# Corv/CUDA-GMM-MPI

Measured on NVIDIA H100. Metric: EM iterations/sec at N=10M D=24 K=64; E-step HBM GB/s vs roofline, higher is better.
Workload: dtype f32

## Files before the change

cuda-gmm-mpi_b200/csrc/gmm_api.cu:

```cuda
#include <cuda_runtime.h>
#include <dlfcn.h>
#include <fcntl.h>
#include <unistd.h>
#include <nccl.h>

#include <algorithm>
#include <atomic>
#include <chrono>
#include <condition_variable>
#include <functional>
#include <mutex>
#include <cmath>
#include <cstdint>
#include <cstdio>
#include <cstdlib>
#include <cstring>
#include <limits>
#include <string>
#include <thread>
#include <vector>

#include "../../include/gmm.h"
#include "host_math.h"
#include "kernels_simt.cuh"
// ... 2671 lines not shown
    if (!c || !out) return fail(GMM_ERR_ARG, "gmm_get_profile: bad argument");
    cudaStreamSynchronize(c->stream);
    collect_all(c);
    out[0] = c->t_estep.total_ms; out[1] = c->t_mstep.total_ms; out[2] = c->host_const_ms;
    out[3] = c->t_reduce.total_ms; out[4] = c->memcpy_ms + c->t_final.total_ms; out[5] = (double)c->mstep_tensor;
    out[6] = (double)c->iterations; out[7] = (double)c->mstep_simt;
    if (reset) {
        c->t_estep.total_ms = c->t_mstep.total_ms = c->t_reduce.total_ms = c->t_fused.total_ms = 0;
        c->host_const_ms = c->memcpy_ms = 0; c->iterations = 0; c->t_final.total_ms = 0;
        c->mstep_tensor = c->mstep_simt = 0;
        c->fit_reduce_ms = c->fit_seed_ms = c->fit_save_ms = 0;
    }
    return GMM_OK;
}

int gmm_host_pool_selftest(int threads, int jobs, int n) {
    if (threads < 1 || jobs < 1 || n < 0) return fail(GMM_ERR_ARG, "gmm_host_pool_selftest: bad argument");
    HostPool pool(threads);
    std::vector<std::atomic<int>> hits((size_t)(n > 0 ? n : 1));
    for (auto& h : hits) h.store(0);
    for (int j = 0; j < jobs; j++) {
        const int m = (j % 3 == 0) ? n : (j % 3 == 1 ? (n + 1) / 2 : 1);
        const std::function<void(int)> fn = [&](int i) { hits[(size_t)i].fetch_add(1, std::memory_order_relaxed); };
        pool.run(m, fn);
        for (int i = 0; i < n; i++) {
            const int want = i < m ? 1 : 0;
            if (hits[(size_t)i].exchange(0) != want) return fail(GMM_ERR_STATE, "gmm_host_pool_selftest: an item ran the wrong number of times");
        }
        if (j % 64 == 63) pool.resize(1 + (j / 64) % threads);
        if (j % 200 == 199) std::this_thread::sleep_for(std::chrono::milliseconds(6));
// ... 71 lines not shown
```

cuda-gmm-mpi_b200/csrc/kernels_tc.cu:

```cuda
#include <cuda.h>
#include <cudaTypedefs.h>
#include <cuda_fp16.h>
#if defined(__F16C__) && defined(__AVX__)
#include <immintrin.h>
#endif
#include <cuda_runtime.h>

#include <cmath>
#include <cstdio>
#include <cstdlib>
#include <cstring>
#include <string>
#include <type_traits>
#include <vector>

#include "host_math.h"
#include "kernels_tc.cuh"
#include "mstep_rows.h"
#include "tc_ptx.cuh"

namespace gmm {

using namespace ptx;

// ... 14 lines not shown
constexpr float kGammaScale = 1024.0f;
constexpr float kGammaMagic = 1.5f * 134217728.0f;

template <int D, int NCL_> struct MCfg {
    static_assert(D % 4 == 0, "tensor M-step: D must be a multiple of 4");
    static_assert(NCL_ == 32 || NCL_ == 64, "tensor M-step: 32 or 64 clusters per CTA");
    static constexpr int NCL = NCL_;
    static constexpr int HPC = 64 / NCL;
    static constexpr int F = 1 + D + D * (D + 1) / 2;
    static constexpr int S = D / 4;
    static constexpr int MT = (4 * ((1 + 2 * S + S * (D / 2) + 7) / 8) * 8 + 127) / 128;
    static constexpr int G_PART = NCL * kTE * 2;
    static constexpr int G_STAGE = 3 * G_PART;
    static constexpr int RAWZ = (D * kTE * 4 + 1023) / 1024 * 1024;
    static constexpr int RAWX = RAWZ + 1024;
    static constexpr int RAWG = NCL * kTE * 4;
    static constexpr int OFF_G = 0;
    static constexpr int OFF_RAWX = OFF_G + kNST * G_STAGE;
    static constexpr int OFF_RAWG = OFF_RAWX + kNRAW * RAWX;
    static constexpr int NCT = MT * 128;
    static constexpr int OFF_RACC = OFF_RAWG + kNRAW * RAWG;
    static constexpr int OFF_BAR = OFF_RACC + 32 * NCT * 4;
    static constexpr int SMEM_BYTES = OFF_BAR + 512;
    static constexpr int THREADS = 128 + NCT;
    static constexpr int REG_LAUNCH = (65536 / THREADS) / 8 * 8 > 255 ? 255 : (65536 / THREADS) / 8 * 8;
    static constexpr int REG_P = MT == 1 ? REG_LAUNCH : 56;
    static constexpr int REG_C = MT == 3 ? 152 : (MT == 2 ? 224 : REG_LAUNCH);
    static_assert(128 * REG_P + NCT * REG_C <= THREADS * REG_LAUNCH, "register pools");
    static_assert(OFF_RAWX % 1024 == 0 && RAWX % 1024 == 0 && RAWZ % 1024 == 0, "SWIZZLE_128B TMA destinations need 1024-byte alignment");
    static_assert(OFF_RAWG % 1024 == 0 && RAWG % 1024 == 0, "SWIZZLE_128B TMA destinations need 1024-byte alignment");
    static_assert(MT <= 3, "feature tiles");
};

// ... 47 lines not shown
        lo[ks][2 * u + 1] = pack_half2(l2, l3);
#endif
    }
}

__device__ __forceinline__ void load_row(uint32_t addr, float2 (&z)[4]) {
#pragma unroll
    for (int p = 0; p < 4; p++) z[p] = lds_f2(addr ^ (uint32_t)(p << 5));
}

template <int NCL>
__device__ __forceinline__ void issue_half(float (&ex)[NCL / 2], float (&rm)[NCL / 2], const uint32_t (&hi)[2][4], const uint32_t (&lo)[2][4],
                                           uint32_t gam, bool new1, bool new2) {
#pragma unroll
    for (int ks = 0; ks < kTE / 16; ks++) {
        const uint64_t hdesc = make_smem_desc(gam + ks * 256,  128,  512);
        const uint64_t ldesc = make_smem_desc(gam + NCL * kTE * 2 + ks * 256, 128, 512);
        const uint64_t sdesc = make_smem_desc(gam + 2 * NCL * kTE * 2 + ks * 256, 128, 512);
#if GMM_MSTEP_CUT == 1
        asm volatile("" ::"r"(hi[ks][0]), "r"(hi[ks][1]), "r"(hi[ks][2]), "r"(hi[ks][3]), "r"(lo[ks][0]), "r"(lo[ks][1]), "r"(lo[ks][2]),
                     "r"(lo[ks][3]), "l"(hdesc), "l"(ldesc), "l"(sdesc));
        (void)ex; (void)rm; (void)new1; (void)new2;
#else
        if constexpr (NCL == 32) {
            wgmma_m64n32k16_rs(ex, hi[ks][0], hi[ks][1], hi[ks][2], hi[ks][3], hdesc, ks > 0 || !new1);
            wgmma_m64n32k16_rs(rm, hi[ks][0], hi[ks][1], hi[ks][2], hi[ks][3], ldesc, ks > 0 || !new2);
            wgmma_m64n32k16_rs(rm, lo[ks][0], lo[ks][1], lo[ks][2], lo[ks][3], sdesc, true);
        } else {
            wgmma_m64n64k16_rs(ex, hi[ks][0], hi[ks][1], hi[ks][2], hi[ks][3], hdesc, ks > 0 || !new1);
            wgmma_m64n64k16_rs(rm, hi[ks][0], hi[ks][1], hi[ks][2], hi[ks][3], ldesc, ks > 0 || !new2);
            wgmma_m64n64k16_rs(rm, lo[ks][0], lo[ks][1], lo[ks][2], lo[ks][3], sdesc, true);
        }
#endif
// ... 5 lines not shown
__device__ __forceinline__ bool chain2_ends(int i, int mt, int nsub) { return ((i + mt) % kChunkSub2) == kChunkSub2 - 1 || i == nsub - 1; }
__device__ __forceinline__ bool chain2_starts(int i, int mt) { return i == 0 || ((i + mt) % kChunkSub2) == 0; }

template <int D, int NCL, bool WT = false>
__global__ void __launch_bounds__(MCfg<D, NCL>::THREADS, 1)
mstep_tc_kernel(const __grid_constant__ CUtensorMap tm_x, const __grid_constant__ CUtensorMap tm_g, int n, int K,
                float* __restrict__ scratch, int events_per_cta, const __grid_constant__ MMagic magic, const int* __restrict__ opmap,
                const float* __restrict__ wts, float w_max, float w_inv) {
    using C = MCfg<D, NCL>;
    constexpr int HPC = C::HPC;
    extern __shared__ __align__(1024) uint8_t smem[];
    uint64_t* bars = reinterpret_cast<uint64_t*>(smem + C::OFF_BAR);
    uint64_t* raw_full = bars;
    uint64_t* raw_empty = bars + kNRAW;
    uint64_t* op_full = bars + 2 * kNRAW;
    uint64_t* op_empty = op_full + kNST;

    const int warp = threadIdx.x >> 5, lane = threadIdx.x & 31;
    const int range = blockIdx.x / (2 / HPC), part = blockIdx.x % (2 / HPC);
    const int e_begin = range * events_per_cta;
    const int e_end = min(n, e_begin + events_per_cta);
    const int nsub = (e_end - e_begin + kTE - 1) / kTE;
    const int k0 = blockIdx.y * NCL;

    for (int i = threadIdx.x; i < kNRAW * 256; i += C::THREADS)
        reinterpret_cast<float*>(smem + C::OFF_RAWX + (i >> 8) * C::RAWX + C::RAWZ)[i & 255] = 1.0f;
    if (threadIdx.x == 0) {
        for (int s = 0; s < kNRAW; s++) { mbar_init(&raw_full[s], 1); mbar_init(&raw_empty[s], 3 + 4 * C::MT); }
        for (int s = 0; s < kNST; s++) { mbar_init(&op_full[s], 3); mbar_init(&op_empty[s], 4 * C::MT); }
        fence_mbar_init();
    }
    __syncthreads();

    if (warp < 4) {
        set_regs<C::REG_P, C::REG_LAUNCH>();
        if (warp == 0) {
            const int nbox = min(NCL, K - k0 + kNCL - 1) / kNCL;
            if (elect_one()) {
                for (int i = 0; i < nsub; i++) {
                    const int st = i % kNRAW, ph = (i / kNRAW) & 1;
                    mbar_wait_parked(&raw_empty[st], ph ^ 1, 500);
                    mbar_arrive_expect_tx(&raw_full[st], kTE * D * 4 + nbox * kNCL * kTE * 4);
                    const int e0 = e_begin + i * kTE;
                    tma_load_2d(smem + C::OFF_RAWX + st * C::RAWX, &tm_x, e0, 0, &raw_full[st]);
                    for (int b = 0; b < nbox; b++)
                        tma_load_2d(smem + C::OFF_RAWG + st * C::RAWG + b * kNCL * kTE * 4, &tm_g, e0, k0 + b * kNCL, &raw_full[st]);
                }
            }
        } else {
            const int bt = threadIdx.x - 32;
            constexpr int NITEM = 4 * NCL, NIT = (NITEM + 95) / 96;
            for (int i = 0; i < nsub; i++) {
                const int rs = i % kNRAW, rph = (i / kNRAW) & 1;
                const int os = i % kNST, oph = (i / kNST) & 1;
                [[maybe_unused]] float wv[8];
                if constexpr (WT) {
                    const float4* wp = reinterpret_cast<const float4*>(wts + e_begin + i * kTE + 8 * ((bt & 31) >> 3));
                    const float4 wa = __ldg(wp), wb = __ldg(wp + 1);
                    wv[0] = wa.x; wv[1] = wa.y; wv[2] = wa.z; wv[3] = wa.w; wv[4] = wb.x; wv[5] = wb.y; wv[6] = wb.z; wv[7] = wb.w;
#pragma unroll
                    for (int v = 0; v < 8; v++) wv[v] = wv[v] == w_max ? 1.0f : __fmul_rn(wv[v], w_inv);
                }
                mbar_wait_parked(&raw_full[rs], rph, 200);
                mbar_wait_parked(&op_empty[os], oph ^ 1, 200);
                uint8_t* g_hi = smem + C::OFF_G + os * C::G_STAGE;
                float dep = 0.0f;
#pragma unroll
                for (int u = 0; u < NIT; u++) {
                    const int it = bt + 96 * u;
                    if (it >= NITEM) break;
                    const int kg = it >> 5, l = it & 31;
                    const int k = kg * 8 + (l & 7), ce = l >> 3;
                    const uint8_t* grow = smem + C::OFF_RAWG + rs * C::RAWG + k * (kTE * 4);
                    const float4 a = *reinterpret_cast<const float4*>(grow + (((2 * ce) ^ (k & 7)) << 4));
                    const float4 b = *reinterpret_cast<const float4*>(grow + (((2 * ce + 1) ^ (k & 7)) << 4));
                    float g[8] = {a.x, a.y, a.z, a.w, b.x, b.y, b.z, b.w};
                    dep += a.x + b.x;
                    if constexpr (WT) {
#pragma unroll
                        for (int v = 0; v < 8; v++) g[v] = __fmul_rn(g[v], wv[v]);
                    }
                    float hi[8], lo[8];
#pragma unroll
                    for (int v = 0; v < 8; v++) {
                        hi[v] = __fsub_rn(__fmaf_rn(g[v], kGammaScale, kGammaMagic), kGammaMagic);
// ... 51 lines not shown
            for (int j = 0; j < NCL / 2; j++) { ex[h][j] = 0.0f; rm[h][j] = 0.0f; }
        auto add_to_racc = [&](float (&acc)[HPC][NCL / 2]) {
#pragma unroll
            for (int c = 0; c < 2; c++) {
#pragma unroll
                for (int j = 0; j < 16; j++) {
                    const int q = 16 * c + j;
                    racc[q * C::NCT] += acc[q / (NCL / 2)][q % (NCL / 2)];
                }
                asm volatile("" ::: "memory");
            }
        };
        uint32_t fh[2][2][4], fl[2][2][4];
        float2 za[4];
        int held = -1;
        auto group = [&](int i, auto hc, uint32_t (&gh)[2][4], uint32_t (&gl)[2][4]) {
            constexpr int h = decltype(hc)::value;
            const int rs = i % kNRAW, rph = (i / kNRAW) & 1;
            const int os = i % kNST, oph = (i / kNST) & 1;
            const uint32_t zst = zs0 + rs * C::RAWX;
            const uint32_t gam = smem_u32(smem + C::OFF_G + os * C::G_STAGE);
            const bool new1 = chain_starts(i, mt), new2 = chain2_starts(i, mt);
            if constexpr (h == 0) {
                mbar_wait_parked(&raw_full[rs], rph, 100);
                load_row(zst + fa, za);
            }
            float2 zb0[4], zb1[4];
            load_row(zst + fb[2 * h], zb0);
            load_row(zst + fb[2 * h + 1], zb1);
            build_half(za, zb0, zb1, mg[2 * h], mg[2 * h + 1], gh, gl);
            if constexpr (h == 0) mbar_wait_parked(&op_full[os], oph, 100);
            wgmma_fence();
            issue_half<NCL>(ex[h], rm[h], gh, gl, gam, new1, new2);
            wgmma_commit();
            if constexpr (h == HPC - 1) {
                __syncwarp();
                if (lane == 0) mbar_arrive(&raw_empty[rs]);
            }
            wgmma_wait<1>();
            if constexpr (h == 0) {
                __syncwarp();
                if (lane == 0 && held >= 0) mbar_arrive(&op_empty[held]);
            }
            if constexpr (h == HPC - 1) {
                held = os;
                if (chain_ends(i, mt, nsub)) {
                    wgmma_wait<0>();
                    __syncwarp();
                    if (lane == 0) mbar_arrive(&op_empty[os]);
                    held = -1;
#if GMM_MSTEP_CUT != 3
                    add_to_racc(ex);
                    if (chain2_ends(i, mt, nsub)) add_to_racc(rm);
#endif
                }
            }
        };
        using H0 = std::integral_constant<int, 0>;
        using H1 = std::integral_constant<int, 1>;
        if constexpr (HPC == 2) {
            for (int i = 0; i < nsub; i++) {
                group(i, H0{}, fh[0], fl[0]);
                group(i, H1{}, fh[1], fl[1]);
            }
// ... 14 lines not shown
        add_to_racc(ex);
#endif
        const int nranges = gridDim.x * HPC / 2;
#pragma unroll
        for (int h = 0; h < HPC; h++)
#pragma unroll
            for (int j = 0; j < NCL / 2; j += 2) {
                const int q = h * (NCL / 2) + j;
                const int row = ((hx & 1) + h) * 64 + wq * 16 + gid + 8 * ((j >> 1) & 1);
                const int col = (j >> 2) * 8 + 2 * qd;
                const int ty = blockIdx.y * (NCL / kNCL) + col / kNCL;
                float* dst = scratch + ((((size_t)ty * nranges + range) * C::MT + mt) * 128 + row) * kNCL + col % kNCL;
                *reinterpret_cast<float2*>(dst) = make_float2(racc[q * C::NCT], racc[(q + 1) * C::NCT]);
            }
    }
}

__global__ void standardise_soa_kernel(const float* __restrict__ xs, float* __restrict__ zs, size_t pitch, int n, int D,
                                       const float* __restrict__ shift_f, const float* __restrict__ inv_scale_f) {
    const int d = blockIdx.y;
    const float s = shift_f[d], isc = inv_scale_f[d];
    const float* x = xs + (size_t)d * pitch;
    float* z = zs + (size_t)d * pitch;
    for (long long e = (long long)blockIdx.x * blockDim.x + threadIdx.x; e < n; e += (long long)gridDim.x * blockDim.x)
        z[e] = __fmul_rn(__fsub_rn(x[e], s), isc);
}

__global__ void __launch_bounds__(256)
mstep_tc_finalize_kernel(const float* __restrict__ scratch, int ncta_x, int MT, int K, int F, const int3* __restrict__ rowmap,
                         const double* __restrict__ scale, double* __restrict__ stats, double wscale) {
// ... 464 lines not shown
    bool emap_ok = false;
    uint8_t* d_bimg = nullptr;
    uint8_t* h_bimg = nullptr;
    size_t bimg_bytes = 0;
    uint8_t* d_opnd = nullptr;
    uint8_t* h_opnd = nullptr;
    cudaEvent_t ev_h2d = nullptr;
    bool h2d_pending = false;
    float* d_ck = nullptr;
    float* h_ck = nullptr;
    float* d_den = nullptr;
    int e_ck_len = 0;
    int e_NG = 0;
    int host_threads = 8;
    bool attr_estep = false, attr_mstep = false, attr_score = false;
    double h_shift[GMM_MAX_DIMENSIONS] = {0}, h_scale[GMM_MAX_DIMENSIONS] = {0};
};

static PFN_cuTensorMapEncodeTiled_v12000 encode_fn() {
    static PFN_cuTensorMapEncodeTiled_v12000 fn = nullptr;
    static bool tried = false;
    if (!tried) {
        tried = true;
        void* p = nullptr;
        cudaDriverEntryPointQueryResult q;
        if (cudaGetDriverEntryPoint("cuTensorMapEncodeTiled", &p, cudaEnableDefault, &q) == cudaSuccess && q == cudaDriverEntryPointSuccess)
            fn = reinterpret_cast<PFN_cuTensorMapEncodeTiled_v12000>(p);
    }
    return fn;
}
// ... 644 lines not shown
    return GMM_OK;
}

int tc_launch_score(TcState* t, int K, const TcScoreIo& io, cudaStream_t stream) {
    if (!t || !t->emap_ok) return fail(GMM_ERR_STATE, "tensor scoring not initialised for this shape");
    if (io.n <= 0) return GMM_OK;
    switch (t->D) {
        case 8: return launch_score_d<8>(t, K, io, stream);
        case 16: return launch_score_d<16>(t, K, io, stream);
        case 24: return launch_score_d<24>(t, K, io, stream);
        default: return fail(GMM_ERR_ARG, "tensor scoring: unsupported D");
    }
}

template <int D>
static int launch_mstep_d(TcState* t, int K, const CUtensorMap& tm_x, const CUtensorMap& tm_g, int n, double* d_stats, const float* w,
                          double wscale, cudaStream_t stream) {
    using C32 = MCfg<D, 32>;
    using C64 = MCfg<D, 64>;
    static_assert(C32::SMEM_BYTES <= 232448 && C64::SMEM_BYTES <= 232448, "shared memory budget");
    if (!t->attr_mstep) {
        TC_CUDA_TRY(cudaFuncSetAttribute(mstep_tc_kernel<D, 32>, cudaFuncAttributeMaxDynamicSharedMemorySize, C32::SMEM_BYTES));
        TC_CUDA_TRY(cudaFuncSetAttribute(mstep_tc_kernel<D, 64>, cudaFuncAttributeMaxDynamicSharedMemorySize, C64::SMEM_BYTES));
        TC_CUDA_TRY(cudaFuncSetAttribute(mstep_tc_kernel<D, 32, true>, cudaFuncAttributeMaxDynamicSharedMemorySize, C32::SMEM_BYTES));
        TC_CUDA_TRY(cudaFuncSetAttribute(mstep_tc_kernel<D, 64, true>, cudaFuncAttributeMaxDynamicSharedMemorySize, C64::SMEM_BYTES));
        t->attr_mstep = true;
    }
    const float w_max = (float)wscale, w_inv = (float)(1.0 / wscale);
    int gx = t->num_sms;
    int per = (n + gx - 1) / gx;
    per = (per + kTE - 1) / kTE * kTE;
    gx = (n + per - 1) / per;
    const bool pair = K > 32;
    const int ncl = pair ? 64 : 32;
    const int gy = (K + ncl - 1) / ncl;
    if ((size_t)gx * gy * (ncl / kNCL) * C32::MT * 128 * kNCL > t->scratch_floats) return fail(GMM_ERR_STATE, "tensor M-step scratch too small");
    const dim3 grid(pair ? 2 * gx : gx, gy);
    if (pair) {
        if (w) mstep_tc_kernel<D, 64, true><<<grid, C64::THREADS, C64::SMEM_BYTES, stream>>>(tm_x, tm_g, n, K, t->d_scratch, per, t->magic, t->d_opmap, w, w_max, w_inv);
        else mstep_tc_kernel<D, 64><<<grid, C64::THREADS, C64::SMEM_BYTES, stream>>>(tm_x, tm_g, n, K, t->d_scratch, per, t->magic, t->d_opmap, nullptr, 1.0f, 1.0f);
    } else {
        if (w) mstep_tc_kernel<D, 32, true><<<grid, C32::THREADS, C32::SMEM_BYTES, stream>>>(tm_x, tm_g, n, K, t->d_scratch, per, t->magic, t->d_opmap, w, w_max, w_inv);
        else mstep_tc_kernel<D, 32><<<grid, C32::THREADS, C32::SMEM_BYTES, stream>>>(tm_x, tm_g, n, K, t->d_scratch, per, t->magic, t->d_opmap, nullptr, 1.0f, 1.0f);
    }
    TC_CUDA_TRY(cudaGetLastError());
    mstep_tc_finalize_kernel<<<C32::MT * 128, 256, 0, stream>>>(t->d_scratch, gx, C32::MT, K, C32::F, t->d_rowmap, t->d_scale, d_stats,
                                                                w ? wscale : 1.0);
    TC_CUDA_TRY(cudaGetLastError());
    return GMM_OK;
}

static int launch_mstep_any(TcState* t, int K, const CUtensorMap& tm_x, const CUtensorMap& tm_g, int n, double* d_stats, const float* w,
                            double wscale, cudaStream_t stream) {
    if (!t || !t->maps_ok) return fail(GMM_ERR_STATE, "tensor-core M-step not initialised for this shape");
    if (!t->have_shift) return fail(GMM_ERR_STATE, "tensor-core M-step needs gmm_seed (shift/scale) first");
// ... 16 lines not shown

int tc_launch_mstep_on(TcState* t, int K, const float* d_z, const float* d_memb, size_t pitch, int n, double* d_stats, cudaStream_t stream) {
    if (n <= 0) return GMM_OK;
    if (!t || !t->maps_ok) return fail(GMM_ERR_STATE, "tensor-core M-step not initialised for this shape");
    if (t->cmap_z != d_z || t->cmap_g != d_memb || t->cmap_pitch != pitch || t->cmap_n != n) {
        t->cmap_n = -1;
        if (int rc = make_map_2d(&t->tm_cx, d_z, (uint64_t)n, (uint64_t)t->D, (uint64_t)pitch * 4, kTE, (uint32_t)t->D, true)) return rc;
        if (int rc = make_map_2d(&t->tm_cg, d_memb, (uint64_t)n, (uint64_t)t->Kmax, (uint64_t)pitch * 4, kTE, kNCL, true)) return rc;
        t->cmap_z = d_z; t->cmap_g = d_memb; t->cmap_pitch = pitch; t->cmap_n = n;
    }
    return launch_mstep_any(t, K, t->tm_cx, t->tm_cg, n, d_stats, nullptr, 1.0, stream);
}

const float* tc_shift_f(const TcState* t) { return t && t->have_shift ? t->d_shift_f : nullptr; }
const float* tc_inv_scale_f(const TcState* t) { return t && t->have_shift ? t->d_inv_scale_f : nullptr; }
float tc_mstep_zbound(const TcState* t) {
    float zb = 0.f;
    if (t)
        for (int d = 0; d < t->D; d++) zb = std::fmax(zb, t->zmax[d]);
    return zb;
}

}
```

cuda-gmm-mpi_b200/csrc/kernels_tc.cuh:

```cuda
#pragma once
#include <cuda_runtime.h>
#include "../../include/gmm.h"

namespace gmm {

struct TcState;

bool tc_mstep_supported(int D, int K);
bool tc_estep_supported(int D, int K);

int  tc_create(TcState** out, const float* d_x_aos, const float* d_x_soa, int n, int D, int Kmax, float* d_memb, size_t memb_pitch,
               int num_sms, cudaStream_t stream);
void tc_destroy(TcState*);
void tc_set_host_threads(TcState*, int n);
int  tc_set_shift_scale(TcState*, double* shift, const double* scale, const double* xmin, const double* xmax, cudaStream_t stream);
bool tc_mstep_ready(const TcState*);
bool tc_estep_range_ok(const TcState*);
int  tc_upload_params(TcState*, const clusters_t* host, int K, cudaStream_t stream);
int  tc_params_begin(TcState*, int K, cudaStream_t stream);
int  tc_params_padded(const TcState*, int K);
int  tc_params_cluster(TcState*, const clusters_t* host, int k, int K);
int  tc_params_cluster_w(TcState*, const clusters_t* host, int k, int K, const double* W);
int  tc_params_commit(TcState*, int K, int bad, cudaStream_t stream);
int  tc_launch_estep(TcState*, int K, double* d_ll, cudaStream_t stream, const float* d_w = nullptr);
// ... 11 lines not shown
};
int  tc_launch_score(TcState*, int K, const TcScoreIo& io, cudaStream_t stream);
bool tc_finalize_supported(const TcState*, int K);
size_t tc_param_set_floats(int Kmax, int D);
size_t tc_param_set_off(int Kmax, int D, int which);
int  tc_launch_finalize(TcState*, int K, const double* d_stats, const float* d_avgvar, float* d_set, double* d_ll, int* d_bad, int iter,
                        int fault_iter, cudaStream_t stream);
int  tc_launch_mstep(TcState*, int K, double* d_stats, cudaStream_t stream, const float* d_w = nullptr, double wscale = 1.0);

int  tc_launch_estep_on(TcState*, int K, const float* d_x_aos, int n, float* d_memb, size_t pitch, float* d_den, double* d_ll,
                        cudaStream_t stream);
int  tc_launch_mstep_on(TcState*, int K, const float* d_z, const float* d_memb, size_t pitch, int n, double* d_stats, cudaStream_t stream);
const float* tc_shift_f(const TcState*);
const float* tc_inv_scale_f(const TcState*);
float tc_mstep_zbound(const TcState*);

}
```

cuda-gmm-mpi_b200/csrc/tc_ptx.cuh:

```cuda
#pragma once
#include <cuda_runtime.h>
#include <cstdint>

namespace gmm { namespace ptx {

__device__ __forceinline__ uint32_t smem_u32(const void* p) {
    return static_cast<uint32_t>(__cvta_generic_to_shared(p));
}

__device__ __forceinline__ void mbar_init(uint64_t* bar, uint32_t count) {
    asm volatile("mbarrier.init.shared::cta.b64 [%0], %1;" ::"r"(smem_u32(bar)), "r"(count) : "memory");
}
__device__ __forceinline__ void fence_mbar_init() {
    asm volatile("fence.mbarrier_init.release.cluster;" ::: "memory");
}
__device__ __forceinline__ void mbar_arrive(uint64_t* bar) {
    asm volatile("mbarrier.arrive.shared::cta.b64 _, [%0];" ::"r"(smem_u32(bar)) : "memory");
}
__device__ __forceinline__ void mbar_arrive_after(uint64_t* bar, float dep) {
    asm volatile(
        "{\n\t.reg .pred p;\n\t.reg .b32 cnt;\n\t"
        "setp.ne.b32 p, %1, 0xff800001;\n\t"
        "selp.b32 cnt, 1, 2, p;\n\t"
        "mbarrier.arrive.shared::cta.b64 _, [%0], cnt;\n\t}"
// ... 12 lines not shown
    return ok != 0;
}
__device__ __forceinline__ void mbar_wait(uint64_t* bar, uint32_t parity) {
    while (!mbar_try_wait(bar, parity)) {}
}
__device__ __forceinline__ void mbar_wait_parked(uint64_t* bar, uint32_t parity, uint32_t ns) {
    uint32_t ok = 0;
    while (!ok) {
        asm volatile(
            "{\n\t.reg .pred p;\n\t"
            "mbarrier.try_wait.parity.shared::cta.b64 p, [%1], %2, %3;\n\t"
            "selp.u32 %0, 1, 0, p;\n\t}"
            : "=r"(ok) : "r"(smem_u32(bar)), "r"(parity), "r"(ns) : "memory");
    }
}
__device__ __forceinline__ void fence_proxy_async_smem() {
    asm volatile("fence.proxy.async.shared::cta;" ::: "memory");
}

__device__ __forceinline__ void tma_load_1d(void* smem_dst, const void* gmem_src, uint32_t bytes, uint64_t* bar) {
    asm volatile(
        "cp.async.bulk.shared::cluster.global.mbarrier::complete_tx::bytes [%0], [%1], %2, [%3];"
        ::"r"(smem_u32(smem_dst)), "l"(gmem_src), "r"(bytes), "r"(smem_u32(bar)) : "memory");
}

__device__ __forceinline__ uint64_t make_smem_desc(uint32_t saddr, uint32_t lbo_bytes, uint32_t sbo_bytes) {
    uint64_t d = 0;
    d |= (uint64_t)((saddr >> 4) & 0x3FFF);
    d |= (uint64_t)((lbo_bytes >> 4) & 0x3FFF) << 16;
    d |= (uint64_t)((sbo_bytes >> 4) & 0x3FFF) << 32;
// ... 71 lines not shown
```

cuda-gmm-mpi_b200/engine.py:

```python
import ctypes as C
import os
import subprocess

import numpy as np

from .clusters import Clusters, clusters_t

_HERE = os.path.dirname(os.path.abspath(__file__))
_FP = C.POINTER(C.c_float)
_DP = C.POINTER(C.c_double)
_IP = C.POINTER(C.c_int)
_CP = C.POINTER(clusters_t)

PATH_AUTO, PATH_SIMT, PATH_TENSOR = 0, 1, 2
VB_DIRICHLET_PROCESS, VB_DIRICHLET_DISTRIBUTION = 0, 1


class gmm_vb_prior(C.Structure):
    _fields_ = [("weight_prior_type", C.c_int), ("weight_concentration", C.c_double), ("mean_precision", C.c_double),
                ("dof", C.c_double), ("mean", _DP), ("covariance", _DP), ("reg_covar", C.c_double)]


class gmm_vb_posterior(C.Structure):
    _fields_ = [("weights", _DP), ("weight_concentration", _DP), ("mean_precision", _DP), ("dof", _DP), ("mean_prior", _DP),
# ... 67 lines not shown
    L.gmm_comm_init.argtypes = [C.c_void_p, C.c_int, C.c_int, C.c_char_p]
    L.gmm_comm_rank.argtypes = [C.c_void_p, _IP, _IP]
    L.gmm_set_option.argtypes = [C.c_void_p, C.c_char_p, C.c_double]
    L.gmm_seed.argtypes = [C.c_void_p, C.c_int, _CP]
    L.gmm_seed_kmeans.argtypes = [C.c_void_p, C.c_int, C.c_int, C.c_ulonglong, _CP, _FP, _IP, _DP]
    L.gmm_set_clusters.argtypes = [C.c_void_p, C.c_int, _CP]
    L.gmm_set_weights.argtypes = [C.c_void_p, C.c_void_p, _DP]
    L.gmm_get_clusters.argtypes = [C.c_void_p, C.c_int, _CP, C.c_int]
    L.gmm_estep.argtypes = [C.c_void_p, C.c_int, _FP]
    L.gmm_mstep.argtypes = [C.c_void_p, C.c_int]
    L.gmm_constants.argtypes = [C.c_void_p, C.c_int]
    L.gmm_em.argtypes = [C.c_void_p, C.c_int, C.c_int, C.c_int, C.c_float, _FP, _IP]
    L.gmm_em_iterations.argtypes = [C.c_void_p, C.c_int, C.c_int, _FP]
    L.gmm_get_profile.argtypes = [C.c_void_p, _DP, C.c_int]
    L.gmm_get_fit_profile.argtypes = [C.c_void_p, _DP]
    L.gmm_score.argtypes = [C.c_void_p, C.c_int, C.c_void_p, C.c_longlong, C.c_void_p, C.c_void_p, C.c_void_p, _DP]
    L.gmm_get_score_profile.argtypes = [C.c_void_p, _DP, C.c_int]
    L.gmm_score_stats.argtypes = [C.c_void_p, C.c_int, C.c_void_p, C.c_longlong, C.c_void_p, C.c_void_p, C.c_void_p]
    L.gmm_get_score_stats_profile.argtypes = [C.c_void_p, _DP, C.c_int]
    L.gmm_sample.argtypes = [C.c_void_p, C.c_int, C.c_longlong, C.c_ulonglong, C.c_longlong, C.c_void_p, C.c_void_p]
    L.gmm_get_sample_profile.argtypes = [C.c_void_p, _DP, C.c_int]
    L.gmm_condition.argtypes = [C.c_void_p, C.c_int, C.c_void_p, C.c_int, C.c_void_p, C.c_longlong, C.c_void_p, C.c_void_p,
                                C.c_void_p, C.c_void_p, C.c_void_p, _DP]
    L.gmm_get_condition_profile.argtypes = [C.c_void_p, _DP, C.c_int]
    L.gmm_condition_stats.argtypes = [C.c_void_p, C.c_int, C.c_void_p, C.c_int, C.c_void_p, C.c_longlong, C.c_void_p, C.c_void_p,
                                      C.c_void_p]
    L.gmm_get_condition_stats_profile.argtypes = [C.c_void_p, _DP, C.c_int]
    L.gmm_fit.argtypes = [C.c_void_p, C.c_int, C.c_int, C.c_int, C.c_int, _CP, _IP, _FP]
    L.gmm_vb_em.argtypes = [C.c_void_p, C.c_int, C.POINTER(gmm_vb_prior), C.c_int, C.c_int, C.c_double, _CP,
                            C.POINTER(gmm_vb_posterior), _DP, _DP, _IP, _IP]
# ... 225 lines not shown
        _check(self.lib.gmm_em(self.h, K, min_iters, max_iters, epsilon, C.byref(ll), C.byref(it)))
        return ll.value, it.value

    def em_iterations(self, K, iters):
        ll = C.c_float()
        _check(self.lib.gmm_em_iterations(self.h, K, iters, C.byref(ll)))
        return ll.value

    def profile(self, reset=False):
        out = (C.c_double * 8)()
        _check(self.lib.gmm_get_profile(self.h, out, int(reset)))
        keys = ("estep_ms", "mstep_ms", "constants_host_ms", "allreduce_ms", "upload_ms", "mstep_tensor_launches", "iterations",
                "mstep_simt_launches")
        return dict(zip(keys, list(out)[:8]))

    def score(self, K, events, labels=True, max_resp=True, logp=True):
        ev = np.ascontiguousarray(events, np.float32)
        if ev.ndim != 2 or ev.shape[1] != self.D:
            raise ValueError(f"events must be [n][{self.D}], got {ev.shape}")
        n = ev.shape[0]
        lab = np.empty(n, np.int32) if labels else None
        mr = np.empty(n, np.float32) if max_resp else None
        lp = np.empty(n, np.float32) if logp else None
        ptr = lambda a: a.ctypes.data if a is not None and a.size else None
        ll = C.c_double()
        _check(self.lib.gmm_score(self.h, K, ptr(ev), n, ptr(lab), ptr(mr), ptr(lp), C.byref(ll)))
        return lab, mr, lp, ll.value

    def score_profile(self, reset=False):
        out = (C.c_double * 4)()
# ... 111 lines not shown
```

include/gmm.h:

```cpp
#ifndef GMM_B200_H
#define GMM_B200_H

#ifdef __cplusplus
extern "C" {
#endif

typedef struct {
    float* N;
    float* pi;
    float* constant;
    float* avgvar;
    float* means;
    float* R;
    float* Rinv;
    float* memberships;
} clusters_t;

typedef struct gmm_ctx gmm_ctx;

enum {
    GMM_OK = 0,
    GMM_ERR_ARG = 1,
    GMM_ERR_IO = 2,
    GMM_ERR_NOMEM = 3,
// ... 97 lines not shown

int  gmm_vb_em(gmm_ctx*, int K, const gmm_vb_prior* prior, int min_iters, int max_iters, double tol,
               clusters_t* host_out, gmm_vb_posterior* post_out,
               double* lower_bound_out, double* lower_bounds_out ,
               int* iters_out, int* converged_out);

int  gmm_host_vb_finalize(const double* stats, const double* shift, int K, int D, const gmm_vb_prior* prior,
                          clusters_t* out, gmm_vb_posterior* post_out, double* bound_out);

int  gmm_host_digamma(const double* x, double* out, long long n);

int  gmm_get_vb_profile(gmm_ctx*, double out[3], int reset);

int  gmm_get_profile(gmm_ctx*, double out[8], int reset);

int  gmm_get_fit_profile(gmm_ctx*, double out[4]);

int  gmm_fit(gmm_ctx*, int K0, int target_K, int min_iters, int max_iters,
             clusters_t* saved, int* ideal_K, float* min_rissanen);


int  gmm_host_invert(float* data, int n, float* log_det, int use_log10);

long long gmm_stats_len(int K, int D);

int  gmm_host_finalize(const double* stats, const double* shift, int K, int D,
                       clusters_t* inout);

int  gmm_host_pool_selftest(int threads, int jobs, int n);

// ... 19 lines not shown
```

Measured before the change: 136.4.

## Split K=64 M-step gamma conversion across a 2-CTA cluster with DSMEM exchange

```diff
diff --git a/cuda-gmm-mpi_b200/csrc/gmm_api.cu b/cuda-gmm-mpi_b200/csrc/gmm_api.cu
--- a/cuda-gmm-mpi_b200/csrc/gmm_api.cu
+++ b/cuda-gmm-mpi_b200/csrc/gmm_api.cu
@@ -2709,6 +2709,13 @@
     return GMM_OK;
 }
 
+int gmm_get_mstep_pairs_resident(gmm_ctx* c, int* out) {
+    if (!c || !out) return fail(GMM_ERR_ARG, "gmm_get_mstep_pairs_resident: bad argument");
+    CUDA_TRY(cudaSetDevice(c->device));
+    *out = c->tc ? tc_mstep_pairs_resident(c->tc) : 0;
+    return GMM_OK;
+}
+
 int gmm_host_pool_selftest(int threads, int jobs, int n) {
     if (threads < 1 || jobs < 1 || n < 0) return fail(GMM_ERR_ARG, "gmm_host_pool_selftest: bad argument");
     HostPool pool(threads);
diff --git a/cuda-gmm-mpi_b200/csrc/kernels_tc.cu b/cuda-gmm-mpi_b200/csrc/kernels_tc.cu
--- a/cuda-gmm-mpi_b200/csrc/kernels_tc.cu
+++ b/cuda-gmm-mpi_b200/csrc/kernels_tc.cu
@@ -52,9 +52,10 @@
     static constexpr int G_STAGE = 3 * G_PART;
     static constexpr int RAWZ = (D * kTE * 4 + 1023) / 1024 * 1024;
     static constexpr int RAWX = RAWZ + 1024;
-    static constexpr int RAWG = NCL * kTE * 4;
+    static constexpr int RAWG = kNCL * kTE * 4;
     static constexpr int OFF_G = 0;
-    static constexpr int OFF_RAWX = OFF_G + kNST * G_STAGE;
+    static constexpr int NST = NCL == 64 ? 4 : kNST;
+    static constexpr int OFF_RAWX = OFF_G + NST * G_STAGE;
     static constexpr int OFF_RAWG = OFF_RAWX + kNRAW * RAWX;
     static constexpr int NCT = MT * 128;
     static constexpr int OFF_RACC = OFF_RAWG + kNRAW * RAWG;
@@ -132,9 +133,10 @@
                                            uint32_t gam, bool new1, bool new2) {
 #pragma unroll
     for (int ks = 0; ks < kTE / 16; ks++) {
-        const uint64_t hdesc = make_smem_desc(gam + ks * 256,  128,  512);
-        const uint64_t ldesc = make_smem_desc(gam + NCL * kTE * 2 + ks * 256, 128, 512);
-        const uint64_t sdesc = make_smem_desc(gam + 2 * NCL * kTE * 2 + ks * 256, 128, 512);
+        constexpr uint32_t GOFF = NCL == 64 ? 512 : NCL * kTE * 2, SBO = NCL == 64 ? 1536 : 512;
+        const uint64_t hdesc = make_smem_desc(gam + ks * 256,  128, SBO);
+        const uint64_t ldesc = make_smem_desc(gam + GOFF + ks * 256, 128, SBO);
+        const uint64_t sdesc = make_smem_desc(gam + 2 * GOFF + ks * 256, 128, SBO);
 #if GMM_MSTEP_CUT == 1
         asm volatile("" ::"r"(hi[ks][0]), "r"(hi[ks][1]), "r"(hi[ks][2]), "r"(hi[ks][3]), "r"(lo[ks][0]), "r"(lo[ks][1]), "r"(lo[ks][2]),
                      "r"(lo[ks][3]), "l"(hdesc), "l"(ldesc), "l"(sdesc));
@@ -170,7 +172,7 @@
     uint64_t* raw_full = bars;
     uint64_t* raw_empty = bars + kNRAW;
     uint64_t* op_full = bars + 2 * kNRAW;
-    uint64_t* op_empty = op_full + kNST;
+    uint64_t* op_empty = op_full + C::NST;
 
     const int warp = threadIdx.x >> 5, lane = threadIdx.x & 31;
     const int range = blockIdx.x / (2 / HPC), part = blockIdx.x % (2 / HPC);
@@ -179,28 +181,95 @@
     const int nsub = (e_end - e_begin + kTE - 1) / kTE;
     const int k0 = blockIdx.y * NCL;
 
+    constexpr bool PAIR = NCL == 64;
+
     for (int i = threadIdx.x; i < kNRAW * 256; i += C::THREADS)
         reinterpret_cast<float*>(smem + C::OFF_RAWX + (i >> 8) * C::RAWX + C::RAWZ)[i & 255] = 1.0f;
     if (threadIdx.x == 0) {
         for (int s = 0; s < kNRAW; s++) { mbar_init(&raw_full[s], 1); mbar_init(&raw_empty[s], 3 + 4 * C::MT); }
-        for (int s = 0; s < kNST; s++) { mbar_init(&op_full[s], 3); mbar_init(&op_empty[s], 4 * C::MT); }
+        for (int s = 0; s < C::NST; s++) { mbar_init(&op_full[s], PAIR ? 1 : 3); mbar_init(&op_empty[s], 4 * C::MT * (PAIR ? 2 : 1)); }
         fence_mbar_init();
     }
-    __syncthreads();
+    if constexpr (PAIR) cluster_sync();
+    else __syncthreads();
+    [[maybe_unused]] const uint32_t peer_delta = PAIR ? mapa_u32(smem_u32(smem), (uint32_t)part ^ 1u) - smem_u32(smem) : 0u;
 
     if (warp < 4) {
         set_regs<C::REG_P, C::REG_LAUNCH>();
         if (warp == 0) {
-            const int nbox = min(NCL, K - k0 + kNCL - 1) / kNCL;
+            const int kb = k0 + kNCL * part;
+            const bool live = kb < K;
             if (elect_one()) {
                 for (int i = 0; i < nsub; i++) {
                     const int st = i % kNRAW, ph = (i / kNRAW) & 1;
                     mbar_wait_parked(&raw_empty[st], ph ^ 1, 500);
-                    mbar_arrive_expect_tx(&raw_full[st], kTE * D * 4 + nbox * kNCL * kTE * 4);
+                    mbar_arrive_expect_tx(&raw_full[st], kTE * D * 4 + (live ? kNCL * kTE * 4 : 0));
                     const int e0 = e_begin + i * kTE;
                     tma_load_2d(smem + C::OFF_RAWX + st * C::RAWX, &tm_x, e0, 0, &raw_full[st]);
-                    for (int b = 0; b < nbox; b++)
-                        tma_load_2d(smem + C::OFF_RAWG + st * C::RAWG + b * kNCL * kTE * 4, &tm_g, e0, k0 + b * kNCL, &raw_full[st]);
+                    if (live) tma_load_2d(smem + C::OFF_RAWG + st * C::RAWG, &tm_g, e0, kb, &raw_full[st]);
+                }
+            }
+        } else if constexpr (PAIR) {
+            const int bt = threadIdx.x - 32;
+            constexpr int NITEM = 256, NIT = 3;
+            for (int i = 0; i < nsub; i++) {
+                const int rs = i % kNRAW, rph = (i / kNRAW) & 1;
+                const int os = i % C::NST, oph = (i / C::NST) & 1;
+                [[maybe_unused]] float wv[NIT][4];
+                if constexpr (WT) {
+#pragma unroll
+                    for (int u = 0; u < NIT; u++) {
+                        const int l = (bt + 96 * u) & 63;
+                        const float4 w4 = __ldg(reinterpret_cast<const float4*>(wts + e_begin + i * kTE + 8 * (l >> 4) + 4 * (l & 1)));
+                        wv[u][0] = w4.x; wv[u][1] = w4.y; wv[u][2] = w4.z; wv[u][3] = w4.w;
+#pragma unroll
+                        for (int v = 0; v < 4; v++) wv[u][v] = wv[u][v] == w_max ? 1.0f : __fmul_rn(wv[u][v], w_inv);
+                    }
+                }
+                mbar_wait_parked(&raw_full[rs], rph, 200);
+                mbar_wait_parked(&op_empty[os], oph ^ 1, 200);
+                const uint32_t g_st = smem_u32(smem + C::OFF_G + os * C::G_STAGE);
+                const uint8_t* graw = smem + C::OFF_RAWG + rs * C::RAWG;
+                float dep = 0.0f;
+#pragma unroll
+                for (int u = 0; u < NIT; u++) {
+                    const int it = bt + 96 * u;
+                    if (it >= NITEM) break;
+#if GMM_MSTEP_CUT == 5
+                    break;
+#endif
+                    const int kg = it >> 6, l = it & 63;
+                    const int kk = (l >> 1) & 7;
+                    const float4 a = *reinterpret_cast<const float4*>(graw + (kg * 8 + kk) * (kTE * 4) + (((l >> 4) * 2 + (l & 1)) ^ kk) * 16);
+                    float g[4] = {a.x, a.y, a.z, a.w};
+                    dep += a.x;
+                    if constexpr (WT) {
+#pragma unroll
+                        for (int v = 0; v < 4; v++) g[v] = __fmul_rn(g[v], wv[u][v]);
+                    }
+                    float hi[4], lo[4];
+#pragma unroll
+                    for (int v = 0; v < 4; v++) {
+                        hi[v] = __fsub_rn(__fmaf_rn(g[v], kGammaScale, kGammaMagic), kGammaMagic);
+                        lo[v] = __fmaf_rn(g[v], kGammaScale, -hi[v]);
+                    }
+                    const uint32_t off = g_st + (4 * part + kg) * 1536 + l * 8;
+                    const uint32_t h0 = pack_half2(hi[0], hi[1]), h1 = pack_half2(hi[2], hi[3]);
+                    const uint32_t l0 = pack_half2(lo[0], lo[1]), l1 = pack_half2(lo[2], lo[3]);
+                    const uint32_t s0 = pack_half2(g[0] * kGammaScale, g[1] * kGammaScale), s1 = pack_half2(g[2] * kGammaScale, g[3] * kGammaScale);
+                    st_shared_v2(off, h0, h1);
+                    st_shared_v2(off + 512, l0, l1);
+                    st_shared_v2(off + 1024, s0, s1);
+                }
+                __syncwarp();
+                if (lane == 0) mbar_arrive_after(&raw_empty[rs], dep);
+                else asm volatile("" ::"f"(dep));
+                fence_proxy_async_smem();
+                asm volatile("bar.sync 1, 96;" ::: "memory");
+                if (bt == 0) {
+                    const uint32_t half = g_st + 6144 * part;
+                    bulk_copy_to_peer(half + peer_delta, half, 6144, smem_u32(&op_full[os]) + peer_delta);
+                    mbar_arrive_expect_tx(&op_full[os], 6144);
                 }
             }
         } else {
@@ -208,7 +277,7 @@
             constexpr int NITEM = 4 * NCL, NIT = (NITEM + 95) / 96;
             for (int i = 0; i < nsub; i++) {
                 const int rs = i % kNRAW, rph = (i / kNRAW) & 1;
-                const int os = i % kNST, oph = (i / kNST) & 1;
+                const int os = i % C::NST, oph = (i / C::NST) & 1;
                 [[maybe_unused]] float wv[8];
                 if constexpr (WT) {
                     const float4* wp = reinterpret_cast<const float4*>(wts + e_begin + i * kTE + 8 * ((bt & 31) >> 3));
@@ -225,6 +294,11 @@
                 for (int u = 0; u < NIT; u++) {
                     const int it = bt + 96 * u;
                     if (it >= NITEM) break;
+#if GMM_MSTEP_CUT == 4
+                    if (it >= 4 * kNCL) break;
+#elif GMM_MSTEP_CUT == 5
+                    break;
+#endif
                     const int kg = it >> 5, l = it & 31;
                     const int k = kg * 8 + (l & 7), ce = l >> 3;
                     const uint8_t* grow = smem + C::OFF_RAWG + rs * C::RAWG + k * (kTE * 4);
@@ -306,10 +380,14 @@
         uint32_t fh[2][2][4], fl[2][2][4];
         float2 za[4];
         int held = -1;
+        auto release_op = [&](int s) {
+            mbar_arrive(&op_empty[s]);
+            if constexpr (PAIR) mbar_arrive_remote(smem_u32(&op_empty[s]) + peer_delta);
+        };
         auto group = [&](int i, auto hc, uint32_t (&gh)[2][4], uint32_t (&gl)[2][4]) {
             constexpr int h = decltype(hc)::value;
             const int rs = i % kNRAW, rph = (i / kNRAW) & 1;
-            const int os = i % kNST, oph = (i / kNST) & 1;
+            const int os = i % C::NST, oph = (i / C::NST) & 1;
             const uint32_t zst = zs0 + rs * C::RAWX;
             const uint32_t gam = smem_u32(smem + C::OFF_G + os * C::G_STAGE);
             const bool new1 = chain_starts(i, mt), new2 = chain2_starts(i, mt);
@@ -321,7 +399,9 @@
             load_row(zst + fb[2 * h], zb0);
             load_row(zst + fb[2 * h + 1], zb1);
             build_half(za, zb0, zb1, mg[2 * h], mg[2 * h + 1], gh, gl);
-            if constexpr (h == 0) mbar_wait_parked(&op_full[os], oph, 100);
+            if constexpr (h == 0) {
+                mbar_wait_parked(&op_full[os], oph, 100);
+            }
             wgmma_fence();
             issue_half<NCL>(ex[h], rm[h], gh, gl, gam, new1, new2);
             wgmma_commit();
@@ -332,14 +412,14 @@
             wgmma_wait<1>();
             if constexpr (h == 0) {
                 __syncwarp();
-                if (lane == 0 && held >= 0) mbar_arrive(&op_empty[held]);
+                if (lane == 0 && held >= 0) release_op(held);
             }
             if constexpr (h == HPC - 1) {
                 held = os;
                 if (chain_ends(i, mt, nsub)) {
                     wgmma_wait<0>();
                     __syncwarp();
-                    if (lane == 0) mbar_arrive(&op_empty[os]);
+                    if (lane == 0) release_op(os);
                     held = -1;
 #if GMM_MSTEP_CUT != 3
                     add_to_racc(ex);
@@ -384,6 +464,7 @@
                 *reinterpret_cast<float2*>(dst) = make_float2(racc[q * C::NCT], racc[(q + 1) * C::NCT]);
             }
     }
+    if constexpr (PAIR) cluster_sync();
 }
 
 __global__ void standardise_soa_kernel(const float* __restrict__ xs, float* __restrict__ zs, size_t pitch, int n, int D,
@@ -878,6 +959,7 @@
     int e_NG = 0;
     int host_threads = 8;
     bool attr_estep = false, attr_mstep = false, attr_score = false;
+    int mstep_pairs = 0;
     double h_shift[GMM_MAX_DIMENSIONS] = {0}, h_scale[GMM_MAX_DIMENSIONS] = {0};
 };
 
@@ -1552,31 +1634,61 @@
 }
 
 template <int D>
+static int mstep_attrs_d(TcState* t) {
+    using C32 = MCfg<D, 32>;
+    using C64 = MCfg<D, 64>;
+    static_assert(C32::SMEM_BYTES <= 232448 && C64::SMEM_BYTES <= 232448, "shared memory budget");
+    if (t->attr_mstep) return GMM_OK;
+    TC_CUDA_TRY(cudaFuncSetAttribute(mstep_tc_kernel<D, 32>, cudaFuncAttributeMaxDynamicSharedMemorySize, C32::SMEM_BYTES));
+    TC_CUDA_TRY(cudaFuncSetAttribute(mstep_tc_kernel<D, 64>, cudaFuncAttributeMaxDynamicSharedMemorySize, C64::SMEM_BYTES));
+    TC_CUDA_TRY(cudaFuncSetAttribute(mstep_tc_kernel<D, 32, true>, cudaFuncAttributeMaxDynamicSharedMemorySize, C32::SMEM_BYTES));
+    TC_CUDA_TRY(cudaFuncSetAttribute(mstep_tc_kernel<D, 64, true>, cudaFuncAttributeMaxDynamicSharedMemorySize, C64::SMEM_BYTES));
+    cudaLaunchAttribute ca{};
+    ca.id = cudaLaunchAttributeClusterDimension;
+    ca.val.clusterDim.x = 2; ca.val.clusterDim.y = 1; ca.val.clusterDim.z = 1;
+    cudaLaunchConfig_t cfg{};
+    cfg.gridDim = dim3(2 * t->num_sms, 1);
+    cfg.blockDim = dim3(C64::THREADS);
+    cfg.dynamicSmemBytes = C64::SMEM_BYTES;
+    cfg.attrs = &ca;
+    cfg.numAttrs = 1;
+    TC_CUDA_TRY(cudaOccupancyMaxActiveClusters(&t->mstep_pairs, mstep_tc_kernel<D, 64>, &cfg));
+    t->attr_mstep = true;
+    return GMM_OK;
+}
+
+template <int D>
 static int launch_mstep_d(TcState* t, int K, const CUtensorMap& tm_x, const CUtensorMap& tm_g, int n, double* d_stats, const float* w,
                           double wscale, cudaStream_t stream) {
     using C32 = MCfg<D, 32>;
     using C64 = MCfg<D, 64>;
-    static_assert(C32::SMEM_BYTES <= 232448 && C64::SMEM_BYTES <= 232448, "shared memory budget");
-    if (!t->attr_mstep) {
-        TC_CUDA_TRY(cudaFuncSetAttribute(mstep_tc_kernel<D, 32>, cudaFuncAttributeMaxDynamicSharedMemorySize, C32::SMEM_BYTES));
-        TC_CUDA_TRY(cudaFuncSetAttribute(mstep_tc_kernel<D, 64>, cudaFuncAttributeMaxDynamicSharedMemorySize, C64::SMEM_BYTES));
-        TC_CUDA_TRY(cudaFuncSetAttribute(mstep_tc_kernel<D, 32, true>, cudaFuncAttributeMaxDynamicSharedMemorySize, C32::SMEM_BYTES));
-        TC_CUDA_TRY(cudaFuncSetAttribute(mstep_tc_kernel<D, 64, true>, cudaFuncAttributeMaxDynamicSharedMemorySize, C64::SMEM_BYTES));
-        t->attr_mstep = true;
-    }
+    if (int rc = mstep_attrs_d<D>(t)) return rc;
     const float w_max = (float)wscale, w_inv = (float)(1.0 / wscale);
+    const bool pair = K > 32;
     int gx = t->num_sms;
+    if (pair && t->mstep_pairs > 0 && 2 * t->mstep_pairs < gx) gx = 2 * t->mstep_pairs;
     int per = (n + gx - 1) / gx;
     per = (per + kTE - 1) / kTE * kTE;
     gx = (n + per - 1) / per;
-    const bool pair = K > 32;
     const int ncl = pair ? 64 : 32;
     const int gy = (K + ncl - 1) / ncl;
     if ((size_t)gx * gy * (ncl / kNCL) * C32::MT * 128 * kNCL > t->scratch_floats) return fail(GMM_ERR_STATE, "tensor M-step scratch too small");
     const dim3 grid(pair ? 2 * gx : gx, gy);
     if (pair) {
-        if (w) mstep_tc_kernel<D, 64, true><<<grid, C64::THREADS, C64::SMEM_BYTES, stream>>>(tm_x, tm_g, n, K, t->d_scratch, per, t->magic, t->d_opmap, w, w_max, w_inv);
-        else mstep_tc_kernel<D, 64><<<grid, C64::THREADS, C64::SMEM_BYTES, stream>>>(tm_x, tm_g, n, K, t->d_scratch, per, t->magic, t->d_opmap, nullptr, 1.0f, 1.0f);
+        cudaLaunchAttribute ca{};
+        ca.id = cudaLaunchAttributeClusterDimension;
+        ca.val.clusterDim.x = 2; ca.val.clusterDim.y = 1; ca.val.clusterDim.z = 1;
+        cudaLaunchConfig_t cfg{};
+        cfg.gridDim = grid;
+        cfg.blockDim = dim3(C64::THREADS);
+        cfg.dynamicSmemBytes = C64::SMEM_BYTES;
+        cfg.stream = stream;
+        cfg.attrs = &ca;
+        cfg.numAttrs = 1;
+        if (w) TC_CUDA_TRY(cudaLaunchKernelEx(&cfg, mstep_tc_kernel<D, 64, true>, tm_x, tm_g, n, K, t->d_scratch, per, t->magic,
+                                              (const int*)t->d_opmap, w, w_max, w_inv));
+        else TC_CUDA_TRY(cudaLaunchKernelEx(&cfg, mstep_tc_kernel<D, 64>, tm_x, tm_g, n, K, t->d_scratch, per, t->magic,
+                                            (const int*)t->d_opmap, (const float*)nullptr, 1.0f, 1.0f));
     } else {
         if (w) mstep_tc_kernel<D, 32, true><<<grid, C32::THREADS, C32::SMEM_BYTES, stream>>>(tm_x, tm_g, n, K, t->d_scratch, per, t->magic, t->d_opmap, w, w_max, w_inv);
         else mstep_tc_kernel<D, 32><<<grid, C32::THREADS, C32::SMEM_BYTES, stream>>>(tm_x, tm_g, n, K, t->d_scratch, per, t->magic, t->d_opmap, nullptr, 1.0f, 1.0f);
@@ -1623,6 +1735,20 @@
 
 const float* tc_shift_f(const TcState* t) { return t && t->have_shift ? t->d_shift_f : nullptr; }
 const float* tc_inv_scale_f(const TcState* t) { return t && t->have_shift ? t->d_inv_scale_f : nullptr; }
+int tc_mstep_pairs_resident(TcState* t) {
+    if (!t) return 0;
+    int rc = GMM_OK;
+    switch (t->D) {
+        case 4: rc = mstep_attrs_d<4>(t); break;
+        case 8: rc = mstep_attrs_d<8>(t); break;
+        case 12: rc = mstep_attrs_d<12>(t); break;
+        case 16: rc = mstep_attrs_d<16>(t); break;
+        case 20: rc = mstep_attrs_d<20>(t); break;
+        case 24: rc = mstep_attrs_d<24>(t); break;
+        default: return 0;
+    }
+    return rc == GMM_OK ? t->mstep_pairs : 0;
+}
 float tc_mstep_zbound(const TcState* t) {
     float zb = 0.f;
     if (t)
diff --git a/cuda-gmm-mpi_b200/csrc/kernels_tc.cuh b/cuda-gmm-mpi_b200/csrc/kernels_tc.cuh
--- a/cuda-gmm-mpi_b200/csrc/kernels_tc.cuh
+++ b/cuda-gmm-mpi_b200/csrc/kernels_tc.cuh
@@ -49,5 +49,6 @@
 const float* tc_shift_f(const TcState*);
 const float* tc_inv_scale_f(const TcState*);
 float tc_mstep_zbound(const TcState*);
+int tc_mstep_pairs_resident(TcState*);
 
 }
diff --git a/cuda-gmm-mpi_b200/csrc/tc_ptx.cuh b/cuda-gmm-mpi_b200/csrc/tc_ptx.cuh
--- a/cuda-gmm-mpi_b200/csrc/tc_ptx.cuh
+++ b/cuda-gmm-mpi_b200/csrc/tc_ptx.cuh
@@ -50,6 +50,25 @@
             : "=r"(ok) : "r"(smem_u32(bar)), "r"(parity), "r"(ns) : "memory");
     }
 }
+__device__ __forceinline__ uint32_t mapa_u32(uint32_t saddr, uint32_t rank) {
+    uint32_t r;
+    asm volatile("mapa.shared::cluster.u32 %0, %1, %2;" : "=r"(r) : "r"(saddr), "r"(rank));
+    return r;
+}
+__device__ __forceinline__ void cluster_sync() {
+    asm volatile("barrier.cluster.arrive.release;\n\tbarrier.cluster.wait.acquire;" ::: "memory");
+}
+__device__ __forceinline__ void mbar_arrive_remote(uint32_t cluster_addr) {
+    asm volatile("mbarrier.arrive.shared::cluster.b64 _, [%0];" ::"r"(cluster_addr) : "memory");
+}
+__device__ __forceinline__ void bulk_copy_to_peer(uint32_t dst, uint32_t src, uint32_t bytes, uint32_t bar) {
+    asm volatile("cp.async.bulk.shared::cluster.shared::cta.mbarrier::complete_tx::bytes [%0], [%1], %2, [%3];"
+                 ::"r"(dst), "r"(src), "r"(bytes), "r"(bar) : "memory");
+}
+__device__ __forceinline__ void st_shared_v2(uint32_t saddr, uint32_t a, uint32_t b) {
+    asm volatile("st.shared.v2.b32 [%0], {%1, %2};" ::"r"(saddr), "r"(a), "r"(b) : "memory");
+}
+
 __device__ __forceinline__ void fence_proxy_async_smem() {
     asm volatile("fence.proxy.async.shared::cta;" ::: "memory");
 }
diff --git a/cuda-gmm-mpi_b200/engine.py b/cuda-gmm-mpi_b200/engine.py
--- a/cuda-gmm-mpi_b200/engine.py
+++ b/cuda-gmm-mpi_b200/engine.py
@@ -105,6 +105,8 @@
     L.gmm_em_iterations.argtypes = [C.c_void_p, C.c_int, C.c_int, _FP]
     L.gmm_get_profile.argtypes = [C.c_void_p, _DP, C.c_int]
     L.gmm_get_fit_profile.argtypes = [C.c_void_p, _DP]
+    if hasattr(L, "gmm_get_mstep_pairs_resident"):
+        L.gmm_get_mstep_pairs_resident.argtypes = [C.c_void_p, _IP]
     L.gmm_score.argtypes = [C.c_void_p, C.c_int, C.c_void_p, C.c_longlong, C.c_void_p, C.c_void_p, C.c_void_p, _DP]
     L.gmm_get_score_profile.argtypes = [C.c_void_p, _DP, C.c_int]
     L.gmm_score_stats.argtypes = [C.c_void_p, C.c_int, C.c_void_p, C.c_longlong, C.c_void_p, C.c_void_p, C.c_void_p]
@@ -360,6 +362,13 @@
                 "mstep_simt_launches")
         return dict(zip(keys, list(out)[:8]))
 
+    def mstep_pairs_resident(self):
+        if not hasattr(self.lib, "gmm_get_mstep_pairs_resident"):
+            return None
+        pairs = C.c_int()
+        _check(self.lib.gmm_get_mstep_pairs_resident(self.h, C.byref(pairs)))
+        return pairs.value
+
     def score(self, K, events, labels=True, max_resp=True, logp=True):
         ev = np.ascontiguousarray(events, np.float32)
         if ev.ndim != 2 or ev.shape[1] != self.D:
diff --git a/include/gmm.h b/include/gmm.h
--- a/include/gmm.h
+++ b/include/gmm.h
@@ -135,6 +135,8 @@
 
 int  gmm_get_profile(gmm_ctx*, double out[8], int reset);
 
+int  gmm_get_mstep_pairs_resident(gmm_ctx*, int* out);
+
 int  gmm_get_fit_profile(gmm_ctx*, double out[4]);
 
 int  gmm_fit(gmm_ctx*, int K0, int target_K, int min_iters, int max_iters,
```

New measurement: 139.7, median of 6. +2.4%, better.
